# FaspDevTeam/faspsolver

Hardware: AMD Instinct MI355X
Metric: AMG-PCG solve DOF/s (3D 7-pt Poisson 256^3, classical AMG V(1,1) w-Jacobi + PCG, rtol 1e-8) (higher is better)
Workload: dtype f64

## Files before the change

faspsolver_amd/__init__.py:

```python
import ctypes as C
import os
import subprocess

import numpy as np

from . import _types as T
from ._types import *

_HERE = os.path.dirname(os.path.abspath(__file__))
LIB_PATH = os.environ.get("FASP_HIP_LIB") or os.path.join(_HERE, "libfasp_hip.so")
_lib = None

EXPORTS = [
    "fasp_param_amg_init", "fasp_param_solver_init", "fasp_solver_dcsr_krylov_amg",
    "fasp_blas_dcsr_mxv", "fasp_blas_dcsr_aAxpy", "fasp_blas_darray_dotprod",
    "fasp_blas_darray_norm2", "fasp_blas_darray_norminf", "fasp_blas_darray_axpy",
    "fasp_blas_darray_axpby", "fasp_smoother_dcsr_jacobi",
    "fasp_blas_dbsr_mxv", "fasp_blas_dbsr_aAxpy", "fasp_dbsr_getdiaginv", "fasp_smoother_dbsr_jacobi1",
    "fasp_solver_dbsr_pcg", "fasp_solver_dbsr_pbcgs", "fasp_solver_dbsr_pgmres", "fasp_solver_dbsr_pvgmres",
    "fasp_solver_dbsr_pvfgmres", "fasp_hip_bsr_precond_setup", "fasp_hip_bsr_precond_fct", "fasp_hip_bsr_precond_free",
    "fasp_hip_param_input", "fasp_fwrapper_dcsr_krylov_amg_", "fasp_dcsrvec_read2", "fasp_dvec_read",
    "fasp_dbsr_read", "fasp_dcoo_read", "fasp_dcoo_read1", "fasp_dcoo_shift_read", "fasp_dmtx_read", "fasp_dmtxsym_read", "fasp_dvec_write", "fasp_dcsr_write_coo", "fasp_dcsrvec_write2", "fasp_fwrapper_dcsr_amg_", "fasp_fwrapper_dbsr_krylov_amg_", "fasp_hip_free_bsr", "fasp_hip_comm_selftest", "fasp_hip_amg_kernel_info", "fasp_hip_coarse_kernel_info", "fasp_hip_bsr_coarse_kernel_info", "fasp_hip_coding_selftest", "fasp_solver_amg", "fasp_solver_famg", "fasp_hip_amg_solve", "fasp_precond_diag", "fasp_precond_dbsr_diag", "fasp_solver_dcsr_itsolver", "fasp_solver_dcsr_krylov", "fasp_solver_dcsr_krylov_diag", "fasp_solver_dbsr_itsolver", "fasp_solver_dbsr_krylov", "fasp_solver_dbsr_krylov_diag", "fasp_hip_mxv_csr", "fasp_hip_mxv_bsr", "fasp_solver_matfree_init", "fasp_solver_pcg", "fasp_solver_pbcgs", "fasp_solver_pgcg", "fasp_solver_pminres", "fasp_solver_pgmres", "fasp_solver_pvgmres", "fasp_solver_pvfgmres", "fasp_solver_itsolver", "fasp_solver_krylov", "fasp_solver_dcsr_pcg", "fasp_solver_dcsr_pminres", "fasp_solver_dcsr_pgcg", "fasp_solver_dcsr_pgcr", "fasp_solver_dcsr_pbcgs", "fasp_solver_dcsr_pgmres", "fasp_solver_dcsr_pvgmres",
    "fasp_solver_dcsr_pvfgmres", "fasp_hip_precond_setup", "fasp_hip_precond_fct", "fasp_hip_precond_free",
    "fasp_hip_time_bsr_mxv", "fasp_solver_dbsr_krylov_amg", "fasp_hip_bsr_amg_create", "fasp_hip_bsr_amg_create_host",
# ... 1 lines not shown
    "fasp_hip_bsr_amg_get_diaginv", "fasp_hip_bsr_solve",
    "fasp_hip_set_device", "fasp_hip_device_count", "fasp_hip_device_identity", "fasp_hip_available",
    "fasp_hip_amg_create", "fasp_hip_amg_create_host", "fasp_hip_amg_upload",
    "fasp_hip_amg_destroy", "fasp_hip_amg_num_levels", "fasp_hip_amg_get_matrix",
    "fasp_hip_amg_get_cfmark", "fasp_hip_solve", "fasp_hip_set_rhs", "fasp_hip_set_guess",
    "fasp_hip_solve_resident", "fasp_hip_get_solution", "fasp_hip_device_synchronize",
    "fasp_hip_precond_amg",
    "fasp_hip_poisson7pt", "fasp_hip_aniso27pt", "fasp_hip_free_system", "fasp_hip_time_kernel", "fasp_hip_measure_ceilings", "fasp_hip_amg_publish", "fasp_hip_amg_attach", "fasp_hip_amg_unpublish",
    "fasp_precond_setup", "fasp_precond_amg", "fasp_precond_famg", "fasp_precond_amli", "fasp_precond_namli", "fasp_amg_data_create", "fasp_amg_data_free", "fasp_param_amg_to_prec", "fasp_param_prec_to_amg", "fasp_mem_free", "fasp_mem_calloc", "fasp_dvec_alloc", "fasp_dvec_set", "fasp_dvec_free", "fasp_dvec_create", "fasp_dcsr_create", "fasp_dcsr_free", "fasp_smoother_dcsr_gs", "fasp_smoother_dcsr_sor", "fasp_smoother_dcsr_L1diag",
    "fasp_hip_tune", "fasp_hip_comm_unique_id", "fasp_hip_comm_init", "fasp_hip_comm_finalize",
    "fasp_hip_comm_rank", "fasp_hip_comm_size", "fasp_hip_version", "fasp_hip_comm_init_shm",
    "fasp_hip_dist_plan", "fasp_hip_dist_level_info", "fasp_hip_dist_get_matrix",
    "fasp_hip_dist_get_list",
    "fasp_blas_dcsr_vmv", "fasp_blas_dcsr_mxv_agg", "fasp_blas_dcsr_aAxpy_agg", "fasp_blas_darray_ax",
    "fasp_blas_darray_axpyz", "fasp_blas_darray_norm1", "fasp_darray_cp", "fasp_darray_set", "fasp_dvec_isnan",
    "fasp_hip_time_matrix", "fasp_hip_bsr_dist_info", "fasp_hip_seq_schedule_selftest", "fasp_hip_seq_chain_selftest", "fasp_hip_cluster_order", "fasp_hip_permute_csr", "fasp_hip_comm_init_ipc", "fasp_hip_comm_stats", "fasp_hip_comm_timing", "fasp_hip_estream_selftest",
    "fasp_param_ilu_init", "fasp_ilu_data_create", "fasp_ilu_data_free", "fasp_mem_iludata_check", "fasp_ilu_dcsr_setup",
    "fasp_precond_ilu", "fasp_precond_ilu_forward", "fasp_precond_ilu_backward", "fasp_solver_dcsr_krylov_ilu",
    "fasp_solver_dcsr_krylov_ilu_M", "fasp_smoother_dcsr_ilu", "fasp_fwrapper_dcsr_krylov_ilu_",
    "fasp_hip_ilu_resident_count", "fasp_hip_ilu_time",
    "fasp_ilu_dbsr_setup", "fasp_precond_dbsr_ilu", "fasp_solver_dbsr_krylov_ilu", "fasp_smoother_dbsr_ilu",
    "fasp_fwrapper_dbsr_krylov_ilu_",
]


def build(verbose=False):
    cmd = ["make", "-C", os.path.join(_HERE, "csrc")]
    if not verbose:
        cmd.insert(1, "-s")
    subprocess.run(cmd, check=True)

# ... 520 lines not shown
```

faspsolver_amd/csrc/device_csr.hip.h:

```cpp

struct DevCSR {
    int     row = 0, col = 0, nnz = 0;
    int*    ia  = nullptr;
    int*    ja  = nullptr;
    double* val = nullptr;
    int*    dpos = nullptr;
    bool    dup_diag = false;
    bool    sorted = false;
    int     lanes = 8;
    int     kind = 0;
    int     tile_rows = 256;
    int     wrows = 64, wcap = 512;
    unsigned char* code = nullptr;
    int*    rowbase = nullptr;
    int*    doff = nullptr;
    double* dval = nullptr;
    unsigned short* pat = nullptr;
    int*    pstart = nullptr;
    int*    plen = nullptr;
    int*    poff = nullptr;
    double* pval = nullptr;
    int     npat = 0, npent = 0;
    unsigned short* ja16 = nullptr;
    int*            jbase = nullptr;
    int     nxrows = -1;
    int     plane = 0;
    int     win_lo = 0, win_hi = -1;
    unsigned short* lja16 = nullptr;
    int*    tptr = nullptr;
    int*    tcols = nullptr;
    long long ntcols = 0;
    const int* bridge = nullptr;
    double*    bscratch = nullptr;
    int        bridge_dir = 0;
    int*       es_tab = nullptr;
    unsigned short* es_ja16 = nullptr;
    double*    es_part = nullptr;
    int        es_W = 0, es_nc = 0;
    void    release()
    {
        if (es_tab) (void)hipFree(es_tab);
        if (es_part) (void)hipFree(es_part);
        if (es_ja16) (void)hipFree(es_ja16);
        es_tab = nullptr; es_part = nullptr; es_ja16 = nullptr; es_W = es_nc = 0;
        if (bscratch) (void)hipFree(bscratch);
        bscratch = nullptr; bridge = nullptr; bridge_dir = 0;
        if (lja16) (void)hipFree(lja16);
        if (tptr) (void)hipFree(tptr);
        if (tcols) (void)hipFree(tcols);
        lja16 = nullptr; tptr = nullptr; tcols = nullptr;
        nxrows = -1;
        if (ja16) (void)hipFree(ja16);
        ja16 = nullptr;
        if (jbase) (void)hipFree(jbase);
        jbase = nullptr;
// ... 576 lines not shown
        }
        if (pend_r >= 0 && pend_kb < e1w) {
            const int w0 = pend_kb >= e0w ? w : T.hw0[(size_t)w];
            if (w0 < 0 || w0 > w || T.np[(size_t)w0] < 2 || w0 + T.np[(size_t)w0] - 1 <= w) return -8;
            if (++parts[(size_t)w0] == T.np[(size_t)w0]) return -9;
        }
    }
    for (int r = 0; r < nrow; ++r) {
        if (done[(size_t)r] != 1) return -10;
        if (covered[(size_t)r] != (long long)ia[r + 1] - ia[r]) return -11;
    }
    for (int w = 0; w < T.W; ++w)
        if (parts[(size_t)w] != T.np[(size_t)w]) return -12;
    if (info) info[2] = (int)cut_rows;
    return 0;
}

static int upload_csr(const HostCSR& H, DevCSR& D)
{
    D.row = H.row; D.col = H.col; D.nnz = H.nnz;
    HIPCK(hipMalloc(&D.ia, sizeof(int) * ((size_t)H.row + 1)));
    HIPCK(hipMalloc(&D.ja, sizeof(int) * std::max<size_t>(H.nnz, 1)));
    HIPCK(hipMalloc(&D.val, sizeof(double) * (std::max<size_t>(H.nnz, 1) + 2)));
    HIPCK(hipMemsetAsync(D.val + std::max<size_t>(H.nnz, 1), 0, sizeof(double) * 2, g_ctx.stream));
    HIPCK(hipMemcpyAsync(D.ia, H.ia.data(), sizeof(int) * ((size_t)H.row + 1), hipMemcpyHostToDevice, g_ctx.stream));
    pick_kernel(D);
    auto upload_plain = [&]() -> int {
        HIPCK(hipMemcpyAsync(D.ja, H.ja.data(), sizeof(int) * (size_t)H.nnz, hipMemcpyHostToDevice, g_ctx.stream));
        HIPCK(hipMemcpyAsync(D.val, H.val.data(), sizeof(double) * (size_t)H.nnz, hipMemcpyHostToDevice, g_ctx.stream));
        return 0;
// ... 111 lines not shown
        }
        lap("row sort");
        HIPCK(hipMemcpy(D.ja, sj.data(), sizeof(int) * (size_t)H.nnz, hipMemcpyHostToDevice));
        HIPCK(hipMemcpy(D.val, sv.data(), sizeof(double) * (size_t)H.nnz, hipMemcpyHostToDevice));
        lap("memcpy");
        if (square && D.kind == 2) {
            HIPCK(hipMalloc(&D.dpos, sizeof(int) * (size_t)std::max(H.row, 1)));
            HIPCK(hipMemcpy(D.dpos, dp.data(), sizeof(int) * (size_t)H.row, hipMemcpyHostToDevice));
        }
        D.sorted = true;
        if (upload_ja16(D, H.ia.data(), sj.data()) < 0) return ERROR_ALLOC_MEM;
        return build_estream(H.ia.data(), H.row, H.nnz, D);
    }
    if (upload_plain() < 0) return ERROR_ALLOC_MEM;
    if (D.kind == 2 && !g_oneshot_upload && build_xtile(H, D) < 0) return ERROR_ALLOC_MEM;
    if (upload_ja16(D, H.ia.data(), H.ja.data()) < 0) return ERROR_ALLOC_MEM;
    return build_estream(H.ia.data(), H.row, H.nnz, D);
}

struct Tuning { int gen2 = 2, ws2_bpc = 3, maxgrid = -1, xcd = 16, nt = 1, kind = -1, lanes = -1, wrows = -1, wcap = -1, compress = 1, rpl = -1, lds_tab = 1, xcd_pat = 64, spcg_batch = 16, small_lds = 1, ja16 = 1, spcg_fused = 1, spcg_grid = 0, spcg_persist = 1, split_rows = 0, gs_multicolor = 0, seq_flow = 1, seq_strip_kb = 0, seq_jobs = 1, seq_spine = 1, seq_grid = 0, seq_chain = 1, seq_chain_n1 = 0, seq_chain_grid = 0, seq_chain_ref = 0, seq_test_hang = 0, seq_rest_lanes = 0, local_square = 1, fuse_zr = 1, fuse_presmooth = 1, seq_lanes = 0, xtile = 1, rp5_max = 45, rp_bpc = 5, rp_xcd = -1, rp_strip = 2, spcg_test_hang = 0, small_onewave = 4, lazy_coarse = 1, rp_stream = -1, renumber = 1, renumber_chunk = 262144, pcg_dev_beta = 1, spcg_spec = 1, ev_every = 4, pcg_fold = 1, seq_chain_touch = 8, seq_chain_touch_t1 = 1, seq_zero_skip = 1, estream = 1, es_dbg = 0, ilu_form = -1; };
static Tuning g_tune;

template <class K>
static int resident_blocks_per_cu(K kernel)
{
    static std::vector<std::pair<const void*, int>> cache;
    const void* key = reinterpret_cast<const void*>(kernel);
    for (const auto& e : cache)
        if (e.first == key) return e.second;
    int nb = 0;
    if (hipOccupancyMaxActiveBlocksPerMultiprocessor(&nb, kernel, BLOCK, 0) != hipSuccess || nb < 1) nb = 4;
    nb = std::min(nb, 8);
    cache.emplace_back(key, nb);
    return nb;
}

template <class K>
static int launch_persistent(K kernel, int ntiles, CsrArgs& a, int blocks_per_cu = 0)
{
    int cap = (blocks_per_cu > 0 ? std::min(blocks_per_cu, resident_blocks_per_cu(kernel)) : resident_blocks_per_cu(kernel)) * g_ctx.num_cu;
    if (g_tune.maxgrid > 0) cap = g_tune.maxgrid;
    cap = std::min(cap, MAXGRID);
    int grid = std::min(cap, ntiles);
    grid = std::max(8, (grid + 7) / 8 * 8);
    hipLaunchKernelGGL(kernel, dim3(grid), dim3(BLOCK), 0, g_ctx.stream, a);
    return grid;
}

template <int OP>
static int launch_rowpat5(CsrArgs& a)
{
    if constexpr (OP == OP_JACOBI || OP == OP_L1DIAG) { (void)a; return 0; }
    else return launch_persistent(k_csr_rowpat5<OP>, a.ntiles, a, 5);
}

constexpr int WIN_ALIGN = DIST_WIN_ALIGN;
struct RowWin { int lo = 0, hi = -1, goff = 0; };
static bool g_jacobi_dot_done = false;

__global__ __launch_bounds__(BLOCK) void k_bridge_gather(int n, const int* __restrict__ perm, const double* __restrict__ s, double* __restrict__ y,
// ... 124 lines not shown
        const double avg = M.row > 0 ? (double)M.nnz / M.row : 1.0;
        if (avg <= 8.5) return launch_persistent(k_csr_dict8<OP, 8>, a.ntiles, a);
        if (avg <= 20.0) return launch_persistent(k_csr_dict8<OP, 16>, a.ntiles, a);
        return launch_persistent(k_csr_dict8<OP, 24>, a.ntiles, a);
    }
    if (M.kind == 2 && g_tune.gen2 && M.wrows == 64 && M.wcap == 512 && (double)M.nnz <= 7.6 * M.row) {
        if (OP == OP_JACOBI && a.partials) g_jacobi_dot_done = true;
        return launch_persistent(k_csr_lstream<OP, 512>, a.ntiles, a, 4);
    }
    if (M.kind == 2 && g_tune.gen2 >= 2 && g_tune.xtile && M.lja16 && M.wrows == 64 && M.wcap == 512 && (OP != OP_JACOBI || (M.dpos && !M.dup_diag)))
    {
        a.lja16 = M.lja16; a.tptr = M.tptr; a.tcols = M.tcols;
        if (OP == OP_JACOBI && a.partials) g_jacobi_dot_done = true;
        return launch_persistent(k_csr_xtile<OP>, a.ntiles, a, 3);
    }
    if (M.kind == 2 && g_tune.gen2 >= 2 && M.wrows == 64 && M.wcap == 512 && (OP != OP_JACOBI || (M.dpos && !M.dup_diag)))
    {
        if (OP == OP_JACOBI && a.partials) g_jacobi_dot_done = true;
        return launch_persistent(k_csr_wstream2<OP>, a.ntiles, a, g_tune.ws2_bpc);
    }
    if (M.kind == 2) {
        if (M.wrows == 64 && M.wcap == 512) return launch_persistent(k_csr_wstream<OP, 64, 512>, a.ntiles, a);
        if (M.wrows == 64) return launch_persistent(k_csr_wstream<OP, 64, 1024>, a.ntiles, a);
        if (M.wrows == 32 && M.wcap == 512) return launch_persistent(k_csr_wstream<OP, 32, 512>, a.ntiles, a);
        return launch_persistent(k_csr_wstream<OP, 32, 1024>, a.ntiles, a);
    }
    const bool es_rule = g_tune.estream >= 2 || (g_tune.estream == 1 && (double)M.nnz < 256.0 * M.row);
    if (M.es_tab && es_rule && a.ja16 && win.hi < 0 && g_tune.split_rows <= 0 && OP != OP_MXV_DOT && !(OP == OP_JACOBI && (a.partials || M.dup_diag))) {
        const int W = M.es_W, nc = M.es_nc;
        a.es_wc = M.es_tab; a.es_centry = a.es_wc + W + 1; a.es_crow = a.es_centry + nc + 1; a.es_hw0 = a.es_crow + nc + 1; a.es_np = a.es_hw0 + W;
// ... 109 lines not shown
```

faspsolver_amd/csrc/kernels.hip.h:

```cpp
#pragma once

#include <hip/hip_runtime.h>

namespace fasp {

constexpr int BLOCK   = 256;
constexpr int MAXGRID = 2048;

enum RowOp : int {
    OP_MXV = 0,
    OP_RESID,
    OP_ADD,
    OP_SUB,
    OP_AXPY,
    OP_JACOBI,
    OP_L1DIAG,
    OP_MXV_DOT
};

struct CsrArgs {
    int           nrow;
    const int*    ia;
    const int*    ja;
    const double* val;
// ... 30 lines not shown
    double*       zx;
    const double* zdiag;
    double        zomega;
    const unsigned short* lja16;
    const int*    tptr;
    const int*    tcols;
    const int*    es_wc;
    const int*    es_centry;
    const int*    es_crow;
    const int*    es_hw0;
    const int*    es_np;
    const int*    es_cbase;
    const unsigned short* es_ja16;
    double*       es_part;
    unsigned*     es_cnt;
};

__device__ __forceinline__ void zx_store(const CsrArgs& a, int r, double s)
{
    if (a.zx) {
        const double di = a.zdiag[r];
        a.zx[r] = (fabs(di) > 1e-20) ? (1 - a.zomega) * 0.0 + a.zomega * s / di : 0.0;
    }
}

__device__ __forceinline__ double l1_or_jacobi_f(const CsrArgs& a, int r, double t, double d, double xi)
{
    if (a.mark) return a.mark[r] == 0 ? xi + a.omega * t / d : xi;
    return (fabs(d) > 1e-20) ? xi + t / d : xi;
}
// ... 1053 lines not shown
```

faspsolver_amd/csrc/solver.hip:

```cpp
#include <hip/hip_runtime.h>

#include <fcntl.h>
#include <omp.h>
#include <sys/mman.h>
#include <sys/stat.h>
#include <unistd.h>

#include <algorithm>
#include <cfloat>
#include <cmath>
#include <cstdio>
#include <cstdlib>
#include <cstring>
#include <functional>
#include <condition_variable>
#include <memory>
#include <mutex>
#include <string>
#include <thread>
#include <vector>

#include "fasp_comm.h"
#include "fasp_internal.h"
#include "kernels.hip.h"
#include "kernels2.hip.h"
#include "kernels3.hip.h"
#include "small_solvers.hip.h"
#include "seq_split.hip.h"
#include "seq_chain.hip.h"

namespace fasp {

#define HIPCK(expr)                                                                        \
    do {                                                                                   \
        hipError_t e_ = (expr);                                                            \
        if (e_ != hipSuccess) {                                                            \
            std::fprintf(stderr, "### ERROR: fasp_hip: %s failed: %s [%s:%d]\n", #expr,    \
                         hipGetErrorString(e_), __FILE__, __LINE__);                       \
            return ERROR_MISC;                                                             \
        }                                                                                  \
    } while (0)
// ... 480 lines not shown
    const DevLevel& D = h->L[level];
    const DevCSR& M = which == 0 ? D.A : which == 1 ? D.P : D.R;
    if (!M.ia) return ERROR_INPUT_PAR;
    int k = M.kind;
    double bytes = 12.0 * M.nnz + 4.0 * (M.row + 1.0);
    if (M.kind == 0 && M.ja16 && g_tune.ja16) bytes = 10.0 * M.nnz + 4.0 * (M.row + 1.0) + (M.jbase ? 4.0 * M.row : 0.0);
    if (M.code && g_tune.compress) { k = 4; bytes = 1.0 * M.nnz + 4.0 * (M.row + 1.0) + (M.rowbase ? 4.0 * M.row : 0.0); }
    if (M.pat && g_tune.compress) { k = 5; bytes = 2.0 * M.row + (M.rowbase ? 4.0 * M.row : 0.0) + 12.0 * M.npent; }
    if (k == 5 && g_tune.gen2 && M.nxrows >= 0 && !M.rowbase) k = 6;
    else if (k == 5 && g_tune.gen2 >= 2 && M.nxrows >= 0 && M.rowbase && (double)M.nnz <= 0.1 * g_tune.rp5_max * M.row) k = 9;
    if (k == 2 && g_tune.gen2 && M.wrows == 64 && M.wcap == 512 && (double)M.nnz <= 7.6 * M.row) k = 7;
    else if (k == 2 && g_tune.gen2 >= 2 && g_tune.xtile && M.lja16 && M.wrows == 64 && M.wcap == 512) {
        k = 10;
        bytes = 10.0 * M.nnz + 4.0 * (M.row + 1.0) + 4.0 * M.ntcols + 4.0 * ((M.row + 63) / 64 + 1.0);
    }
    else if (k == 2 && g_tune.gen2 >= 2 && M.wrows == 64 && M.wcap == 512) k = 8;
    if (kind) *kind = k;
    if (matrix_bytes) *matrix_bytes = bytes;
    return FASP_SUCCESS;
}

int fasp_hip_coarse_kernel_info(const fasp_hip_amg* h, int* info)
{
    FASP_ENTRY();
    if (!h || !info) return ERROR_INPUT_PAR;
    for (int i = 0; i < 6; ++i) info[i] = h->coarse_kinfo[i];
    info[6] = g_ctx.num_cu; info[7] = 0;
    return FASP_SUCCESS;
}

// ... 1554 lines not shown
    else if (!std::strcmp(key, "seq_chain_ref")) g_tune.seq_chain_ref = value;
    else if (!std::strcmp(key, "seq_spine")) g_tune.seq_spine = value;
    else if (!std::strcmp(key, "seq_partition")) g_seq_partition = value;
    else if (!std::strcmp(key, "fuse_zr")) g_tune.fuse_zr = value;
    else if (!std::strcmp(key, "fuse_presmooth")) g_tune.fuse_presmooth = value;
    else if (!std::strcmp(key, "seq_lanes")) g_tune.seq_lanes = value;
    else if (!std::strcmp(key, "lazy_coarse")) g_tune.lazy_coarse = value;
    else if (!std::strcmp(key, "xtile")) g_tune.xtile = value;
    else if (!std::strcmp(key, "rp5_max")) g_tune.rp5_max = value;
    else if (!std::strcmp(key, "rp_bpc")) g_tune.rp_bpc = value;
    else if (!std::strcmp(key, "rp_stream")) g_tune.rp_stream = value;
    else if (!std::strcmp(key, "renumber")) g_tune.renumber = value;
    else if (!std::strcmp(key, "renumber_chunk")) g_tune.renumber_chunk = value;
    else if (!std::strcmp(key, "time_cold")) g_time_cold = value;
    else if (!std::strcmp(key, "estream")) g_tune.estream = value;
    else if (!std::strcmp(key, "es_dbg")) g_tune.es_dbg = value;
    else if (!std::strcmp(key, "pcg_dev_beta")) g_tune.pcg_dev_beta = value;
    else if (!std::strcmp(key, "seq_chain_touch")) g_tune.seq_chain_touch = value;
    else if (!std::strcmp(key, "seq_chain_touch_t1")) g_tune.seq_chain_touch_t1 = value;
    else if (!std::strcmp(key, "seq_zero_skip")) g_tune.seq_zero_skip = value;
    else if (!std::strcmp(key, "pcg_fold")) g_tune.pcg_fold = value;
    else if (!std::strcmp(key, "spcg_spec")) g_tune.spcg_spec = value;
    else if (!std::strcmp(key, "ev_every")) g_tune.ev_every = value;
    else if (!std::strcmp(key, "rp_xcd")) g_tune.rp_xcd = value;
    else if (!std::strcmp(key, "rp_strip")) g_tune.rp_strip = value;
    else if (!std::strcmp(key, "host_parallel_min")) g_parallel_min_nnz = value;
    else if (!std::strcmp(key, "lanes")) g_tune.lanes = value;
    else if (!std::strcmp(key, "wrows")) g_tune.wrows = value;
    else if (!std::strcmp(key, "wcap")) g_tune.wcap = value;
    else return ERROR_INPUT_PAR;
    return FASP_SUCCESS;
}

int fasp_hip_estream_selftest(const int* ia, int nrow, int nnz, int per_wave, int wmax, int* info)
{
    if (!ia || nrow < 1 || nnz < 1 || per_wave < 8 || wmax < 32) return ERROR_INPUT_PAR;
    return estream_selftest_host(ia, nrow, nnz, per_wave, wmax, info);
}

int fasp_hip_measure_ceilings(double* out, size_t bytes, int reps)
{
    FASP_ENTRY();
    if (!out || bytes < (1u << 20) || reps <= 0) return ERROR_INPUT_PAR;
    if (ctx_init() != FASP_SUCCESS) return ERROR_MISC;
    f64x2_t *p = nullptr, *q = nullptr, *r = nullptr;
// ... 78 lines not shown
        return tot / reps;
    }
    run(); run();
    (void)hipEventRecord(e0, g_ctx.stream);
    for (int i = 0; i < reps; ++i) run();
    (void)hipEventRecord(e1, g_ctx.stream);
    (void)hipEventSynchronize(e1);
    D.b = keep_b; D.x = keep_x;
    float ms = 0.f;
    (void)hipEventElapsedTime(&ms, e0, e1);
    (void)hipEventDestroy(e0); (void)hipEventDestroy(e1);
    return (double)ms / reps;
}


double fasp_hip_time_matrix(const dCSRmat* A, int op, int reps, int* kind_out)
{
    FASP_ENTRY();
    if (!A || reps <= 0 || ctx_init() < 0) return -1.0;
    HostCSR M;
    M.row = A->row; M.col = A->col; M.nnz = A->nnz;
    M.row_aligned = A->col > A->row && std::getenv("FASP_HIP_TIME_ROW_ALIGNED") != nullptr;
    M.ia.view(A->IA, (size_t)A->row + 1); M.ja.view(A->JA, (size_t)std::max(A->nnz, 1)); M.val.view(A->val, (size_t)std::max(A->nnz, 1));
    DevCSR D;
    {
        HostThreads team;
        if (upload_csr(M, D) < 0) { D.release(); return -1.0; }
    }
    const int n = A->row, nc = A->col;
    double *x = nullptr, *y = nullptr, *w = nullptr, *dg = nullptr;
// ... 13 lines not shown
    };
    hipEvent_t e0, e1;
    (void)hipEventCreate(&e0); (void)hipEventCreate(&e1);
    run(); run();
    (void)hipEventRecord(e0, g_ctx.stream);
    for (int i = 0; i < reps; ++i) run();
    (void)hipEventRecord(e1, g_ctx.stream);
    (void)hipEventSynchronize(e1);
    float ms = 0.f;
    (void)hipEventElapsedTime(&ms, e0, e1);
    (void)hipEventDestroy(e0); (void)hipEventDestroy(e1);
    if (kind_out) {
        int k = D.kind;
        if (D.code && g_tune.compress) k = 4;
        if (D.pat && g_tune.compress) k = (D.nxrows >= 0 && g_tune.gen2) ? (D.rowbase ? 9 : 6) : 5;
        *kind_out = k;
    }
    (void)hipFree(x); (void)hipFree(y); (void)hipFree(w); (void)hipFree(dg);
    D.release();
    return (double)ms / reps;
}

}
```

include/fasp_hip_dev.h:

```cpp
#ifndef FASP_HIP_DEV_H
#define FASP_HIP_DEV_H
#include "fasp_hip.h"
#ifdef __cplusplus
extern "C" {
#endif

double fasp_hip_time_kernel(fasp_hip_amg* h, int kind, int level, int reps);
double fasp_hip_time_matrix(const dCSRmat* A, int op, int reps, int* kind_out);
double fasp_hip_seq_schedule_selftest(const dCSRmat* A, const int* seq, int ns, int strip_kb, int lanes, int spine, int* info);
int fasp_hip_cluster_order(const dCSRmat* A, int chunk, int* order);
int fasp_hip_permute_csr(const dCSRmat* A, const int* rperm, const int* cinv, int* ia, int* ja, double* val);
double fasp_hip_seq_chain_selftest(const dCSRmat* A, const int* seq, int ns, int n1_blocks, int form, double w, int* info, double* out_u);
int fasp_hip_measure_ceilings(double* out, size_t bytes, int reps);

int    fasp_hip_ilu_resident_count(void);
double fasp_hip_ilu_time(ILU_data* iludata, int which, int reps, double* info);

int fasp_hip_tune(const char* key, int value);
int fasp_hip_coarse_kernel_info(const fasp_hip_amg* h, int* info);
int fasp_hip_bsr_coarse_kernel_info(const fasp_hip_amg_bsr* h, int* info);

int fasp_hip_comm_stats(double* out8, int reset);
int fasp_hip_comm_timing(int on);

int fasp_hip_dist_plan(fasp_hip_amg* h, int rank, int nranks, int min_rows);
int fasp_hip_dist_level_info(const fasp_hip_amg* h, int level, int* info);
int fasp_hip_dist_get_matrix(const fasp_hip_amg* h, int level, int which, dCSRmat* view);
int fasp_hip_dist_get_list(const fasp_hip_amg* h, int level, int which, ivector* view);
int  fasp_hip_estream_selftest(const int* ia, int nrow, int nnz, int per_wave, int wmax, int* info);
int  fasp_hip_comm_selftest(void);

#ifdef __cplusplus
}
#endif
#endif
```

Baseline: 451.2 million.

## Add value-table compressed SELL-64 format for kind-2 CSR levels

Adds a sliced-ELL (64-row slices) encoding for generic CSR matrices that packs each entry into one 32-bit word: an index into a deduplicated value table plus a column offset from the slice base. A new kernel keeps the value table in LDS and streams the packed codes, aiming to cut the matrix bytes read per SpMV, smoother and residual pass on AMG levels (mainly coarse Galerkin operators with more than about 7.6 nnz per row). It applies only when the number of distinct values and the padding overhead stay within limits. It adds host setup cost for hashing and encoding, uses large blocks with heavy LDS that may limit occupancy, and pads rows to the slice width. Host self-test and per-level operator entry points are added for validation.

```diff
diff --git a/faspsolver_amd/__init__.py b/faspsolver_amd/__init__.py
--- a/faspsolver_amd/__init__.py
+++ b/faspsolver_amd/__init__.py
@@ -39,7 +39,7 @@
     "fasp_hip_dist_get_list",
     "fasp_blas_dcsr_vmv", "fasp_blas_dcsr_mxv_agg", "fasp_blas_dcsr_aAxpy_agg", "fasp_blas_darray_ax",
     "fasp_blas_darray_axpyz", "fasp_blas_darray_norm1", "fasp_darray_cp", "fasp_darray_set", "fasp_dvec_isnan",
-    "fasp_hip_time_matrix", "fasp_hip_bsr_dist_info", "fasp_hip_seq_schedule_selftest", "fasp_hip_seq_chain_selftest", "fasp_hip_cluster_order", "fasp_hip_permute_csr", "fasp_hip_comm_init_ipc", "fasp_hip_comm_stats", "fasp_hip_comm_timing", "fasp_hip_estream_selftest",
+    "fasp_hip_time_matrix", "fasp_hip_bsr_dist_info", "fasp_hip_seq_schedule_selftest", "fasp_hip_seq_chain_selftest", "fasp_hip_cluster_order", "fasp_hip_permute_csr", "fasp_hip_comm_init_ipc", "fasp_hip_comm_stats", "fasp_hip_comm_timing", "fasp_hip_estream_selftest", "fasp_hip_sell_selftest", "fasp_hip_level_op", "fasp_hip_matrix_op",
     "fasp_param_ilu_init", "fasp_ilu_data_create", "fasp_ilu_data_free", "fasp_mem_iludata_check", "fasp_ilu_dcsr_setup",
     "fasp_precond_ilu", "fasp_precond_ilu_forward", "fasp_precond_ilu_backward", "fasp_solver_dcsr_krylov_ilu",
     "fasp_solver_dcsr_krylov_ilu_M", "fasp_smoother_dcsr_ilu", "fasp_fwrapper_dcsr_krylov_ilu_",
diff --git a/faspsolver_amd/csrc/device_csr.hip.h b/faspsolver_amd/csrc/device_csr.hip.h
--- a/faspsolver_amd/csrc/device_csr.hip.h
+++ b/faspsolver_amd/csrc/device_csr.hip.h
@@ -37,8 +37,19 @@
     unsigned short* es_ja16 = nullptr;
     double*    es_part = nullptr;
     int        es_W = 0, es_nc = 0;
+    unsigned*      sell_code = nullptr;
+    int*           sell_meta = nullptr;
+    unsigned char* sell_rlen = nullptr;
+    double*        sell_tab = nullptr;
+    int            sell_nv = 0, sell_obits = 0, sell_nslice = 0;
+    long long      sell_slots = 0;
     void    release()
     {
+        if (sell_code) (void)hipFree(sell_code);
+        if (sell_meta) (void)hipFree(sell_meta);
+        if (sell_rlen) (void)hipFree(sell_rlen);
+        if (sell_tab) (void)hipFree(sell_tab);
+        sell_code = nullptr; sell_meta = nullptr; sell_rlen = nullptr; sell_tab = nullptr; sell_nv = sell_obits = sell_nslice = 0; sell_slots = 0;
         if (es_tab) (void)hipFree(es_tab);
         if (es_part) (void)hipFree(es_part);
         if (es_ja16) (void)hipFree(es_ja16);
@@ -645,6 +656,209 @@
         if (parts[(size_t)w] != T.np[(size_t)w]) return -12;
     if (info) info[2] = (int)cut_rows;
     return 0;
+}
+
+struct SellHost {
+    int nslice = 0, nv = 0, vbits = 0, obits = 0;
+    long long slots = 0;
+    std::vector<int> sptr, sbase;
+    std::vector<unsigned char> rlen;
+    std::vector<double> tab;
+    Buf<unsigned> code;
+    double bytes(int nrow) const { return 4.0 * (double)slots + (double)nrow + 4.0 * (2.0 * nslice + 1.0) + 8.0 * nv; }
+};
+constexpr int SELL_CAP_PERCENT = 125;
+static bool build_sell(const HostCSR& M, SellHost& S, int cap_percent, int* why_not)
+{
+    int dummy = 0;
+    int& why = why_not ? *why_not : dummy;
+    why = 1;
+    const int n = M.row;
+    if (n <= 0 || M.nnz < 4096 || (double)M.nnz > 48.0 * n || (double)M.nnz <= 7.6 * n) return false;
+    if ((long long)M.col >= (1ll << 28)) return false;
+    const int ns = (n + 63) / 64;
+    S.rlen.assign((size_t)n, 0);
+    S.sptr.assign((size_t)ns + 1, 0);
+    int toolong = 0;
+#pragma omp parallel for schedule(static) reduction(+ : toolong)
+    for (int s = 0; s < ns; ++s) {
+        int W = 0;
+        for (int r = s * 64; r < std::min(n, s * 64 + 64); ++r) {
+            const int len = M.ia[r + 1] - M.ia[r];
+            if (len > 255) { ++toolong; continue; }
+            S.rlen[(size_t)r] = (unsigned char)len;
+            W = std::max(W, len);
+        }
+        S.sptr[(size_t)s + 1] = W;
+    }
+    if (toolong) { why = 2; return false; }
+    long long wsum = 0;
+    for (int s = 0; s < ns; ++s) wsum += S.sptr[(size_t)s + 1];
+    S.nslice = ns;
+    S.slots = 64ll * wsum;
+    if (S.slots * 100 > (long long)cap_percent * M.nnz || wsum >= (1ll << 30)) { why = 3; return false; }
+    for (int s = 0; s < ns; ++s) S.sptr[(size_t)s + 1] += S.sptr[(size_t)s];
+    constexpr int VSLOTS = 32768;
+    struct VSet {
+        std::vector<unsigned long long> key;
+        std::vector<long long> cnt;
+        std::vector<int> id;
+        int n = 0;
+        VSet() : key((size_t)VSLOTS, 0ull), cnt((size_t)VSLOTS, 0), id((size_t)VSLOTS, -1) {}
+        static unsigned slot_of(unsigned long long b) { return (unsigned)((b * 0x9E3779B97F4A7C15ull) >> 49); }
+        bool add(unsigned long long b, long long c)
+        {
+            unsigned s = slot_of(b);
+            for (;;) {
+                if (cnt[s] == 0) {
+                    if (n >= SELL_MAXV) return false;
+                    key[s] = b; cnt[s] = c; ++n;
+                    return true;
+                }
+                if (key[s] == b) { cnt[s] += c; return true; }
+                s = (s + 1) & (VSLOTS - 1);
+            }
+        }
+        int slot(unsigned long long b) const
+        {
+            unsigned s = slot_of(b);
+            for (;;) {
+                if (cnt[s] == 0) return -1;
+                if (key[s] == b) return (int)s;
+                s = (s + 1) & (VSLOTS - 1);
+            }
+        }
+    };
+    auto bits_of = [](double v) { unsigned long long b; std::memcpy(&b, &v, 8); return b; };
+    const int nt = std::max(1, std::min(omp_get_max_threads(), n / 4096 + 1));
+    std::vector<VSet*> local((size_t)nt, nullptr);
+    bool fail = false;
+#pragma omp parallel num_threads(nt)
+    {
+        VSet* T = new VSet();
+        local[(size_t)omp_get_thread_num()] = T;
+#pragma omp for schedule(static)
+        for (int r = 0; r < n; ++r) {
+            if (fail) continue;
+            for (int k = M.ia[r]; k < M.ia[r + 1]; ++k)
+                if (!T->add(bits_of(M.val[k]), 1)) { fail = true; break; }
+        }
+    }
+    VSet Gs;
+    for (VSet* T : local) {
+        if (T && !fail)
+            for (int s = 0; s < VSLOTS && !fail; ++s)
+                if (T->cnt[(size_t)s] && !Gs.add(T->key[(size_t)s], T->cnt[(size_t)s])) fail = true;
+        delete T;
+    }
+    if (fail) { why = 4; return false; }
+    std::vector<std::pair<long long, unsigned long long>> order;
+    for (int s = 0; s < VSLOTS; ++s)
+        if (Gs.cnt[(size_t)s]) order.emplace_back(-Gs.cnt[(size_t)s], Gs.key[(size_t)s]);
+    std::sort(order.begin(), order.end());
+    S.nv = (int)order.size();
+    S.tab.resize(order.size());
+    for (size_t i = 0; i < order.size(); ++i) std::memcpy(&S.tab[i], &order[i].second, 8);
+    for (size_t i = 0; i < order.size(); ++i) Gs.id[(size_t)Gs.slot(order[i].second)] = (int)i;
+    S.vbits = 0;
+    while ((1ll << S.vbits) < S.nv) ++S.vbits;
+    S.sbase.assign((size_t)ns, 0);
+    int maxoff = 0;
+#pragma omp parallel for schedule(static) reduction(max : maxoff)
+    for (int s = 0; s < ns; ++s) {
+        const int k0 = M.ia[s * 64], k1 = M.ia[std::min(n, s * 64 + 64)];
+        if (k1 <= k0) continue;
+        int lo = M.ja[k0], hi = lo;
+        for (int k = k0 + 1; k < k1; ++k) { lo = std::min(lo, M.ja[k]); hi = std::max(hi, M.ja[k]); }
+        S.sbase[(size_t)s] = lo;
+        maxoff = std::max(maxoff, hi - lo);
+    }
+    S.obits = 1;
+    while ((1ll << S.obits) <= maxoff) ++S.obits;
+    if (S.vbits + S.obits > 32) { why = 5; return false; }
+    S.code.alloc((size_t)std::max<long long>(S.slots, 1));
+    bool lost = false;
+#pragma omp parallel for schedule(static)
+    for (int s = 0; s < ns; ++s) {
+        const int W = S.sptr[(size_t)s + 1] - S.sptr[(size_t)s], base = S.sbase[(size_t)s];
+        unsigned* cs = S.code.data() + (size_t)S.sptr[(size_t)s] * 64;
+        for (int l = 0; l < 64; ++l) {
+            const int r = s * 64 + l;
+            const int kb = r < n ? M.ia[r] : 0, len = r < n ? M.ia[r + 1] - kb : 0;
+            for (int k = 0; k < len; ++k) {
+                const int sl = Gs.slot(bits_of(M.val[kb + k]));
+                if (sl < 0) { lost = true; continue; }
+                const int id = Gs.id[(size_t)sl];
+                cs[(size_t)k * 64 + l] = ((unsigned)id << S.obits) | (unsigned)(M.ja[kb + k] - base);
+            }
+            for (int k = len; k < W; ++k) cs[(size_t)k * 64 + l] = 0u;
+        }
+    }
+    if (lost) { why = 4; return false; }
+    why = 0;
+    return true;
+}
+
+static void sell_mxv_host(const SellHost& S, int nrow, const double* x, double* y)
+{
+    const unsigned omask = (1u << S.obits) - 1u;
+    for (int s = 0; s < S.nslice; ++s) {
+        const int W = S.sptr[(size_t)s + 1] - S.sptr[(size_t)s], base = S.sbase[(size_t)s];
+        const unsigned* cs = S.code.data() + (size_t)S.sptr[(size_t)s] * 64;
+        double acc[64];
+        for (int l = 0; l < 64; ++l) acc[l] = 0.0;
+        for (int k = 0; k < W; ++k)
+            for (int l = 0; l < 64; ++l) {
+                const int r = s * 64 + l;
+                if (r >= nrow || k >= (int)S.rlen[(size_t)r]) continue;
+                const unsigned c = cs[(size_t)k * 64 + l];
+                acc[l] = acc[l] + S.tab[c >> S.obits] * x[base + (int)(c & omask)];
+            }
+        for (int l = 0; l < 64 && s * 64 + l < nrow; ++l) y[s * 64 + l] = acc[l];
+    }
+}
+static void sell_decode_host(const SellHost& S, int nrow, int* ia, int* ja, double* val)
+{
+    const unsigned omask = (1u << S.obits) - 1u;
+    ia[0] = 0;
+    for (int r = 0; r < nrow; ++r) ia[r + 1] = ia[r] + (int)S.rlen[(size_t)r];
+    for (int r = 0; r < nrow; ++r) {
+        const int s = r >> 6, l = r & 63, base = S.sbase[(size_t)s];
+        const unsigned* cs = S.code.data() + (size_t)S.sptr[(size_t)s] * 64;
+        for (int k = 0; k < (int)S.rlen[(size_t)r]; ++k) {
+            const unsigned c = cs[(size_t)k * 64 + l];
+            ja[ia[r] + k] = base + (int)(c & omask);
+            val[ia[r] + k] = S.tab[c >> S.obits];
+        }
+    }
+}
+
+static int upload_sell(const HostCSR& H, DevCSR& D)
+{
+    static const bool on = !(std::getenv("FASP_HIP_SELL") && std::atoi(std::getenv("FASP_HIP_SELL")) == 0);
+    if (!on) return FASP_SUCCESS;
+    static const bool timing = std::getenv("FASP_HIP_SETUP_TIMING") != nullptr;
+    const double t0 = wall_seconds();
+    SellHost S;
+    int why = 0;
+    const bool ok = build_sell(H, S, SELL_CAP_PERCENT, &why);
+    if (timing) std::printf("        [sell %d x %d, %d nnz] %s (%d) %d values, %d + %d bits, %.3f slots per entry, %.3f s\n", H.row, H.col, H.nnz,
+                            ok ? "coded" : "not coded", why, S.nv, S.vbits, S.obits, (double)S.slots / std::max(H.nnz, 1), wall_seconds() - t0);
+    if (!ok) return FASP_SUCCESS;
+    const size_t ns = (size_t)S.nslice;
+    std::vector<int> meta(2 * ns + 1);
+    std::copy(S.sptr.begin(), S.sptr.end(), meta.begin());
+    std::copy(S.sbase.begin(), S.sbase.end(), meta.begin() + (long)ns + 1);
+    HIPCK(hipMalloc(&D.sell_code, sizeof(unsigned) * (size_t)std::max<long long>(S.slots, 1)));
+    HIPCK(hipMalloc(&D.sell_meta, sizeof(int) * meta.size()));
+    HIPCK(hipMalloc(&D.sell_rlen, (size_t)H.row));
+    HIPCK(hipMalloc(&D.sell_tab, sizeof(double) * (size_t)S.nv));
+    HIPCK(hipMemcpy(D.sell_code, S.code.data(), sizeof(unsigned) * (size_t)S.slots, hipMemcpyHostToDevice));
+    HIPCK(hipMemcpy(D.sell_meta, meta.data(), sizeof(int) * meta.size(), hipMemcpyHostToDevice));
+    HIPCK(hipMemcpy(D.sell_rlen, S.rlen.data(), (size_t)H.row, hipMemcpyHostToDevice));
+    HIPCK(hipMemcpy(D.sell_tab, S.tab.data(), sizeof(double) * (size_t)S.nv, hipMemcpyHostToDevice));
+    D.sell_nv = S.nv; D.sell_obits = S.obits; D.sell_nslice = S.nslice; D.sell_slots = S.slots;
+    return FASP_SUCCESS;
 }
 
 static int upload_csr(const HostCSR& H, DevCSR& D)
@@ -786,11 +1000,12 @@
     }
     if (upload_plain() < 0) return ERROR_ALLOC_MEM;
     if (D.kind == 2 && !g_oneshot_upload && build_xtile(H, D) < 0) return ERROR_ALLOC_MEM;
+    if (D.kind == 2 && compress_enabled() && upload_sell(H, D) < 0) return ERROR_ALLOC_MEM;
     if (upload_ja16(D, H.ia.data(), H.ja.data()) < 0) return ERROR_ALLOC_MEM;
     return build_estream(H.ia.data(), H.row, H.nnz, D);
 }
 
-struct Tuning { int gen2 = 2, ws2_bpc = 3, maxgrid = -1, xcd = 16, nt = 1, kind = -1, lanes = -1, wrows = -1, wcap = -1, compress = 1, rpl = -1, lds_tab = 1, xcd_pat = 64, spcg_batch = 16, small_lds = 1, ja16 = 1, spcg_fused = 1, spcg_grid = 0, spcg_persist = 1, split_rows = 0, gs_multicolor = 0, seq_flow = 1, seq_strip_kb = 0, seq_jobs = 1, seq_spine = 1, seq_grid = 0, seq_chain = 1, seq_chain_n1 = 0, seq_chain_grid = 0, seq_chain_ref = 0, seq_test_hang = 0, seq_rest_lanes = 0, local_square = 1, fuse_zr = 1, fuse_presmooth = 1, seq_lanes = 0, xtile = 1, rp5_max = 45, rp_bpc = 5, rp_xcd = -1, rp_strip = 2, spcg_test_hang = 0, small_onewave = 4, lazy_coarse = 1, rp_stream = -1, renumber = 1, renumber_chunk = 262144, pcg_dev_beta = 1, spcg_spec = 1, ev_every = 4, pcg_fold = 1, seq_chain_touch = 8, seq_chain_touch_t1 = 1, seq_zero_skip = 1, estream = 1, es_dbg = 0, ilu_form = -1; };
+struct Tuning { int gen2 = 2, ws2_bpc = 3, maxgrid = -1, xcd = 16, nt = 1, kind = -1, lanes = -1, wrows = -1, wcap = -1, compress = 1, rpl = -1, lds_tab = 1, xcd_pat = 64, spcg_batch = 16, small_lds = 1, ja16 = 1, spcg_fused = 1, spcg_grid = 0, spcg_persist = 1, split_rows = 0, gs_multicolor = 0, seq_flow = 1, seq_strip_kb = 0, seq_jobs = 1, seq_spine = 1, seq_grid = 0, seq_chain = 1, seq_chain_n1 = 0, seq_chain_grid = 0, seq_chain_ref = 0, seq_test_hang = 0, seq_rest_lanes = 0, local_square = 1, fuse_zr = 1, fuse_presmooth = 1, seq_lanes = 0, xtile = 1, rp5_max = 45, rp_bpc = 5, rp_xcd = -1, rp_strip = 2, spcg_test_hang = 0, small_onewave = 4, lazy_coarse = 1, rp_stream = -1, renumber = 1, renumber_chunk = 262144, pcg_dev_beta = 1, spcg_spec = 1, ev_every = 4, pcg_fold = 1, seq_chain_touch = 8, seq_chain_touch_t1 = 1, seq_zero_skip = 1, estream = 1, es_dbg = 0, ilu_form = -1, sell = 1; };
 static Tuning g_tune;
 
 template <class K>
@@ -816,6 +1031,36 @@
     int grid = std::min(cap, ntiles);
     grid = std::max(8, (grid + 7) / 8 * 8);
     hipLaunchKernelGGL(kernel, dim3(grid), dim3(BLOCK), 0, g_ctx.stream, a);
+    return grid;
+}
+
+static bool sell_active(const DevCSR& M) { return M.sell_code && g_tune.compress && g_tune.sell && g_tune.gen2 >= 2 && !(g_tune.xtile && M.lja16); }
+template <int OP>
+static int launch_sell(const DevCSR& M, CsrArgs& a)
+{
+    a.sell_code = M.sell_code; a.sell_sptr = M.sell_meta; a.sell_sbase = M.sell_meta + M.sell_nslice + 1; a.sell_rlen = M.sell_rlen;
+    a.sell_tab = M.sell_tab; a.sell_nv = M.sell_nv; a.sell_obits = M.sell_obits;
+    const size_t lds = sizeof(double) * ((size_t)M.sell_nv + SELL_NW);
+    static bool attr_set = false;
+    if (!attr_set) {
+        (void)hipFuncSetAttribute(reinterpret_cast<const void*>(k_csr_sell<OP>), hipFuncAttributeMaxDynamicSharedMemorySize, (int)(sizeof(double) * (SELL_MAXV + SELL_NW)));
+        attr_set = true;
+    }
+    static std::vector<std::pair<size_t, int>> cache;
+    int nb = 0;
+    for (const auto& e : cache)
+        if (e.first == lds) nb = e.second;
+    if (nb == 0) {
+        if (hipOccupancyMaxActiveBlocksPerMultiprocessor(&nb, k_csr_sell<OP>, SELL_BLOCK, lds) != hipSuccess || nb < 1) nb = 1;
+        nb = std::min(nb, 2);
+        cache.emplace_back(lds, nb);
+    }
+    int cap = nb * g_ctx.num_cu;
+    if (g_tune.maxgrid > 0) cap = g_tune.maxgrid;
+    cap = std::min(cap, MAXGRID);
+    int grid = std::min(cap, a.ntiles);
+    grid = std::max(8, (grid + 7) / 8 * 8);
+    hipLaunchKernelGGL(k_csr_sell<OP>, dim3(grid), dim3(SELL_BLOCK), lds, g_ctx.stream, a);
     return grid;
 }
 
@@ -970,6 +1215,11 @@
         if (OP == OP_JACOBI && a.partials) g_jacobi_dot_done = true;
         return launch_persistent(k_csr_xtile<OP>, a.ntiles, a, 3);
     }
+    if (M.kind == 2 && sell_active(M) && M.wrows == 64 && M.wcap == 512 && (OP != OP_JACOBI || (M.dpos && !M.dup_diag))) {
+        set_tiles(SELL_BLOCK);
+        if (OP == OP_JACOBI && a.partials) g_jacobi_dot_done = true;
+        return launch_sell<OP>(M, a);
+    }
     if (M.kind == 2 && g_tune.gen2 >= 2 && M.wrows == 64 && M.wcap == 512 && (OP != OP_JACOBI || (M.dpos && !M.dup_diag)))
     {
         if (OP == OP_JACOBI && a.partials) g_jacobi_dot_done = true;
diff --git a/faspsolver_amd/csrc/kernels.hip.h b/faspsolver_amd/csrc/kernels.hip.h
--- a/faspsolver_amd/csrc/kernels.hip.h
+++ b/faspsolver_amd/csrc/kernels.hip.h
@@ -68,6 +68,12 @@
     const unsigned short* es_ja16;
     double*       es_part;
     unsigned*     es_cnt;
+    const unsigned*      sell_code;
+    const int*           sell_sptr;
+    const int*           sell_sbase;
+    const unsigned char* sell_rlen;
+    const double*        sell_tab;
+    int                  sell_nv, sell_obits;
 };
 
 __device__ __forceinline__ void zx_store(const CsrArgs& a, int r, double s)
diff --git a/faspsolver_amd/csrc/kernels4.hip.h b/faspsolver_amd/csrc/kernels4.hip.h
--- /dev/null
+++ b/faspsolver_amd/csrc/kernels4.hip.h
@@ -0,0 +1,113 @@
+#pragma once
+
+#include "kernels2.hip.h"
+
+namespace fasp {
+
+constexpr int SELL_BLOCK = 1024;
+constexpr int SELL_NW    = SELL_BLOCK / 64;
+constexpr int SELL_U     = 8;
+constexpr int SELL_MAXV  = 9216;
+
+template <int OP>
+__global__ __launch_bounds__(SELL_BLOCK, 8) void k_csr_sell(CsrArgs a)
+{
+    if (a.stop && *a.stop) return;
+    extern __shared__ __attribute__((aligned(16))) double sell_lds[];
+    const int lane = threadIdx.x & 63, wave = __builtin_amdgcn_readfirstlane(threadIdx.x >> 6);
+    const int nv = a.sell_nv;
+    for (int i = threadIdx.x; i < nv; i += SELL_BLOCK) sell_lds[i] = a.sell_tab[i];
+    __syncthreads();
+    const double* tab = sell_lds;
+    const int      obits = a.sell_obits;
+    const unsigned omask = (1u << obits) - 1u;
+    const int vmax = tile_vmax(a);
+    const int G = gridDim.x;
+    double dotacc = 0.0;
+
+    auto advance = [&](int& v, int& r0, int& nr) {
+        for (;;) {
+            r0 = -1; nr = 0;
+            if (v >= vmax) return;
+            const int t = tile_of(a, v);
+            v += G;
+            if (t >= a.ntiles) continue;
+            const int rr = (t + a.tile0) * SELL_BLOCK + wave * 64;
+            if (rr >= a.nrow) continue;
+            r0 = rr; nr = min(64, a.nrow - rr);
+            return;
+        }
+    };
+    auto meta = [&](int r0, int nr, int& p0, int& W, int& base, int& len) {
+        p0 = W = base = len = 0;
+        if (r0 < 0) return;
+        const int s = r0 >> 6;
+        p0 = a.sell_sptr[s]; W = a.sell_sptr[s + 1] - p0; base = a.sell_sbase[s];
+        if (lane < nr) len = a.sell_rlen[r0 + lane];
+    };
+    unsigned c[SELL_U];
+    auto load_codes = [&](unsigned* q, int p0, int W, int k0) {
+        const unsigned* cp = a.sell_code + ((size_t)p0 << 6) + lane;
+#pragma unroll
+        for (int u = 0; u < SELL_U; ++u) q[u] = __builtin_nontemporal_load(cp + ((size_t)min(k0 + u, W - 1) << 6));
+    };
+
+    int v = blockIdx.x;
+    int r0A, nrA, p0A, WA, baseA, lenA;
+    advance(v, r0A, nrA);
+    meta(r0A, nrA, p0A, WA, baseA, lenA);
+    if (r0A >= 0 && WA > 0) load_codes(c, p0A, WA, 0);
+    while (r0A >= 0) {
+        int r0B, nrB, p0B, WB, baseB, lenB;
+        advance(v, r0B, nrB);
+        meta(r0B, nrB, p0B, WB, baseB, lenB);
+        const int r = r0A + lane;
+        double acc = ((OP == OP_JACOBI || OP == OP_L1DIAG) && lane < nrA) ? a.b[r] : 0.0;
+        const bool haveB = r0B >= 0 && WB > 0;
+        for (int k0 = 0; k0 < WA; k0 += SELL_U) {
+            int    col[SELL_U];
+            double xv[SELL_U], w[SELL_U];
+#pragma unroll
+            for (int u = 0; u < SELL_U; ++u) col[u] = baseA + (int)(c[u] & omask);
+            unsigned dmask = 0u;
+            if (OP == OP_JACOBI) {
+#pragma unroll
+                for (int u = 0; u < SELL_U; ++u) dmask |= (col[u] == r ? 1u : 0u) << u;
+            }
+#pragma unroll
+            for (int u = 0; u < SELL_U; ++u) xv[u] = a.x[col[u]];
+            unsigned n[SELL_U];
+            const bool more = k0 + SELL_U < WA;
+            load_codes(n, more || !haveB ? p0A : p0B, more || !haveB ? WA : WB, more ? k0 + SELL_U : haveB ? 0 : WA - 1);
+#pragma unroll
+            for (int u = 0; u < SELL_U; ++u) w[u] = tab[c[u] >> obits];
+#pragma unroll
+            for (int u = 0; u < SELL_U; ++u) {
+                const double pr = w[u] * xv[u];
+                bool use = k0 + u < lenA;
+                if (OP == OP_JACOBI) use = use && !((dmask >> u) & 1u);
+                const double nxt = (OP == OP_JACOBI || OP == OP_L1DIAG) ? acc - pr : acc + pr;
+                acc = use ? nxt : acc;
+            }
+#pragma unroll
+            for (int u = 0; u < SELL_U; ++u) c[u] = n[u];
+        }
+        if (WA == 0 && haveB) load_codes(c, p0B, WB, 0);
+        if (lane < nrA) row_epilogue<OP>(a, r, acc, dotacc);
+        r0A = r0B; nrA = nrB; p0A = p0B; WA = WB; baseA = baseB; lenA = lenB;
+    }
+    if (OP == OP_MXV_DOT || (OP == OP_JACOBI && a.partials)) {
+        double* red = sell_lds + nv;
+        const double s = subwave_sum<64>(dotacc);
+        __syncthreads();
+        if (lane == 0) red[wave] = s;
+        __syncthreads();
+        if (threadIdx.x == 0) {
+            double tot = red[0];
+            for (int q = 1; q < SELL_NW; ++q) tot += red[q];
+            a.partials[blockIdx.x] = tot;
+        }
+    }
+}
+
+}
diff --git a/faspsolver_amd/csrc/solver.hip b/faspsolver_amd/csrc/solver.hip
--- a/faspsolver_amd/csrc/solver.hip
+++ b/faspsolver_amd/csrc/solver.hip
@@ -25,6 +25,7 @@
 #include "kernels.hip.h"
 #include "kernels2.hip.h"
 #include "kernels3.hip.h"
+#include "kernels4.hip.h"
 #include "small_solvers.hip.h"
 #include "seq_split.hip.h"
 #include "seq_chain.hip.h"
@@ -535,6 +536,10 @@
         k = 10;
         bytes = 10.0 * M.nnz + 4.0 * (M.row + 1.0) + 4.0 * M.ntcols + 4.0 * ((M.row + 63) / 64 + 1.0);
     }
+    else if (k == 2 && sell_active(M) && M.wrows == 64 && M.wcap == 512) {
+        k = 11;
+        bytes = 4.0 * (double)M.sell_slots + 1.0 * M.row + 4.0 * (2.0 * M.sell_nslice + 1.0) + 8.0 * M.sell_nv;
+    }
     else if (k == 2 && g_tune.gen2 >= 2 && M.wrows == 64 && M.wcap == 512) k = 8;
     if (kind) *kind = k;
     if (matrix_bytes) *matrix_bytes = bytes;
@@ -2119,6 +2124,7 @@
     else if (!std::strcmp(key, "renumber_chunk")) g_tune.renumber_chunk = value;
     else if (!std::strcmp(key, "time_cold")) g_time_cold = value;
     else if (!std::strcmp(key, "estream")) g_tune.estream = value;
+    else if (!std::strcmp(key, "sell")) g_tune.sell = value;
     else if (!std::strcmp(key, "es_dbg")) g_tune.es_dbg = value;
     else if (!std::strcmp(key, "pcg_dev_beta")) g_tune.pcg_dev_beta = value;
     else if (!std::strcmp(key, "seq_chain_touch")) g_tune.seq_chain_touch = value;
@@ -2134,6 +2140,24 @@
     else if (!std::strcmp(key, "wrows")) g_tune.wrows = value;
     else if (!std::strcmp(key, "wcap")) g_tune.wcap = value;
     else return ERROR_INPUT_PAR;
+    return FASP_SUCCESS;
+}
+
+int fasp_hip_sell_selftest(const dCSRmat* A, int cap_percent, int* info, double* bytes, int* ia_out, int* ja_out, double* val_out, const double* x, double* y)
+{
+    if (!A || !info || A->row < 0 || A->nnz < 0) return ERROR_INPUT_PAR;
+    HostCSR M;
+    M.row = A->row; M.col = A->col; M.nnz = A->nnz;
+    M.ia.view(A->IA, (size_t)A->row + 1); M.ja.view(A->JA, (size_t)std::max(A->nnz, 1)); M.val.view(A->val, (size_t)std::max(A->nnz, 1));
+    SellHost S;
+    int why = 0;
+    const bool ok = build_sell(M, S, cap_percent > 0 ? cap_percent : SELL_CAP_PERCENT, &why);
+    info[0] = ok ? 1 : 0; info[1] = why; info[2] = S.nv; info[3] = S.vbits; info[4] = S.obits; info[5] = S.nslice;
+    info[6] = ok ? (int)std::min<long long>(S.slots / 64, 0x7fffffff) : 0; info[7] = SELL_MAXV;
+    if (bytes) *bytes = ok ? S.bytes(M.row) : 0.0;
+    if (!ok) return FASP_SUCCESS;
+    if (ia_out && ja_out && val_out) sell_decode_host(S, M.row, ia_out, ja_out, val_out);
+    if (x && y) sell_mxv_host(S, M.row, x, y);
     return FASP_SUCCESS;
 }
 
@@ -2242,6 +2266,82 @@
 }
 
 
+static int row_op_host(DevLevel& D, int which, int op, const double* x, const double* b, double* y, double* y2, double scalar, double* red)
+{
+    if (which < 0 || which > 2 || op < 0 || op > 8 || !x || !y) return ERROR_INPUT_PAR;
+    const DevCSR& M = which == 0 ? D.A : which == 1 ? D.P : D.R;
+    if (!M.ia || ((op == 5 || op == 6) && which != 0) || ((op == 1 || op >= 5) && !b) || (op == 8 && !y2)) return ERROR_INPUT_PAR;
+    const size_t nr = (size_t)std::max(M.row, 1), nc = (size_t)std::max(M.col, 1);
+    double *dx = nullptr, *db = nullptr, *dy = nullptr, *dy2 = nullptr;
+    int st = FASP_SUCCESS;
+    auto run = [&]() -> int {
+        HIPCK(hipMalloc(&dx, 8 * nc)); HIPCK(hipMalloc(&db, 8 * nr)); HIPCK(hipMalloc(&dy, 8 * nr)); HIPCK(hipMalloc(&dy2, 8 * nr));
+        HIPCK(hipMemcpy(dx, x, 8 * (size_t)M.col, hipMemcpyHostToDevice));
+        HIPCK(hipMemcpy(dy, y, 8 * (size_t)M.row, hipMemcpyHostToDevice));
+        if (b) HIPCK(hipMemcpy(db, b, 8 * (size_t)M.row, hipMemcpyHostToDevice));
+        CsrArgs a{};
+        a.x = dx; a.y = dy; a.b = db;
+        int G = 0;
+        bool have_red = false;
+        switch (op) {
+            case 0: G = launch_csr<OP_MXV>(M, a); break;
+            case 1: G = launch_csr<OP_RESID>(M, a); break;
+            case 2: G = launch_csr<OP_ADD>(M, a); break;
+            case 3: G = launch_csr<OP_SUB>(M, a); break;
+            case 4: a.alpha = scalar; G = launch_csr<OP_AXPY>(M, a); break;
+            case 5:
+                a.diag = D.diag; a.omega = scalar;
+                if (red) { a.partials = g_ctx.d_partials; g_jacobi_dot_done = false; }
+                G = launch_csr<OP_JACOBI>(M, a);
+                have_red = red && g_jacobi_dot_done;
+                g_jacobi_dot_done = false;
+                break;
+            case 6: a.diag = D.l1; a.omega = scalar; G = launch_csr<OP_L1DIAG>(M, a); break;
+            case 7: a.b = nullptr; a.dotv = db; a.partials = g_ctx.d_partials; G = launch_csr<OP_MXV_DOT>(M, a); have_red = red != nullptr; break;
+            default: a.b = nullptr; a.zx = dy2; a.zdiag = db; a.zomega = scalar; G = launch_csr<OP_MXV>(M, a); break;
+        }
+        if (red) *red = std::nan("");
+        if (have_red) {
+            d_finalize(G, 1, 0u, 0, false);
+            if (fetch_red(0, 1, red) < 0) return ERROR_MISC;
+        }
+        HIPCK(hipStreamSynchronize(g_ctx.stream));
+        HIPCK(hipMemcpy(y, dy, 8 * (size_t)M.row, hipMemcpyDeviceToHost));
+        if (op == 8) HIPCK(hipMemcpy(y2, dy2, 8 * (size_t)M.row, hipMemcpyDeviceToHost));
+        return FASP_SUCCESS;
+    };
+    st = run();
+    (void)hipFree(dx); (void)hipFree(db); (void)hipFree(dy); (void)hipFree(dy2);
+    return st;
+}
+
+int fasp_hip_level_op(fasp_hip_amg* h, int level, int which, int op, const double* x, const double* b, double* y, double* y2, double scalar, double* red)
+{
+    FASP_ENTRY();
+    if (!h || level < 0 || level >= (int)h->L.size()) return ERROR_INPUT_PAR;
+    return row_op_host(h->L[level], which, op, x, b, y, y2, scalar, red);
+}
+int fasp_hip_matrix_op(const dCSRmat* A, int op, const double* x, const double* b, double* y, double* y2, double scalar, double* red, int* kind_out)
+{
+    FASP_ENTRY();
+    if (!A || ctx_init() < 0) return ERROR_INPUT_PAR;
+    HostCSR M;
+    M.row = A->row; M.col = A->col; M.nnz = A->nnz;
+    M.ia.view(A->IA, (size_t)A->row + 1); M.ja.view(A->JA, (size_t)std::max(A->nnz, 1)); M.val.view(A->val, (size_t)std::max(A->nnz, 1));
+    DevLevel D;
+    int st;
+    {
+        HostThreads team;
+        st = upload_csr(M, D.A);
+        if (st >= 0 && M.row == M.col) st = upload_diag(M, D);
+    }
+    if (st >= 0 && (op == 5 || op == 6) && !D.diag) st = ERROR_INPUT_PAR;
+    if (st >= 0) st = row_op_host(D, 0, op, x, b, y, y2, scalar, red);
+    if (kind_out) *kind_out = (D.A.kind == 2 && sell_active(D.A)) ? 11 : D.A.kind;
+    free_level(D);
+    return st;
+}
+
 double fasp_hip_time_matrix(const dCSRmat* A, int op, int reps, int* kind_out)
 {
     FASP_ENTRY();
@@ -2285,6 +2385,7 @@
         int k = D.kind;
         if (D.code && g_tune.compress) k = 4;
         if (D.pat && g_tune.compress) k = (D.nxrows >= 0 && g_tune.gen2) ? (D.rowbase ? 9 : 6) : 5;
+        if (k == 2 && sell_active(D) && (double)D.nnz > 7.6 * D.row) k = 11;
         *kind_out = k;
     }
     (void)hipFree(x); (void)hipFree(y); (void)hipFree(w); (void)hipFree(dg);
diff --git a/include/fasp_hip_dev.h b/include/fasp_hip_dev.h
--- a/include/fasp_hip_dev.h
+++ b/include/fasp_hip_dev.h
@@ -28,6 +28,9 @@
 int fasp_hip_dist_get_matrix(const fasp_hip_amg* h, int level, int which, dCSRmat* view);
 int fasp_hip_dist_get_list(const fasp_hip_amg* h, int level, int which, ivector* view);
 int  fasp_hip_estream_selftest(const int* ia, int nrow, int nnz, int per_wave, int wmax, int* info);
+int  fasp_hip_sell_selftest(const dCSRmat* A, int cap_percent, int* info, double* bytes, int* ia_out, int* ja_out, double* val_out, const double* x, double* y);
+int  fasp_hip_level_op(fasp_hip_amg* h, int level, int which, int op, const double* x, const double* b, double* y, double* y2, double scalar, double* red);
+int  fasp_hip_matrix_op(const dCSRmat* A, int op, const double* x, const double* b, double* y, double* y2, double scalar, double* red, int* kind_out);
 int  fasp_hip_comm_selftest(void);
 
 #ifdef __cplusplus
```

Result: faster. 480.7 million, median of 6 (+6.5%).
